# DerEchteKarsten/RayTracer3

Hardware: AMD Instinct MI355X
Metric: Mrays/s (higher is better)
Workload: dtype f32

## Files before the change

### raytracer3_amd/csrc/rt3_device.hpp

```cpp
#pragma once
#include <hip/hip_fp16.h>
#include <hip/hip_runtime.h>
#include <stdint.h>

#define RT3_DEV __device__ __forceinline__

namespace rt3 {

constexpr float kPi = 3.14159265358979323846f;
constexpr float kTau = 6.28318530717958647692f;
constexpr float kInvPi = 0.318309886183790671538f;
constexpr float kHalfPi = 1.57079632679489661923f;
constexpr float kBackgroundDepth = 100000.0f;
constexpr uint32_t kMiss = 0xFFFFFFFFu;
constexpr float kRayTMin = 0.001f;

struct V3 {
    float x, y, z;
};
RT3_DEV V3 v3(float x, float y, float z) { return V3{x, y, z}; }
RT3_DEV V3 operator+(V3 a, V3 b) { return V3{a.x + b.x, a.y + b.y, a.z + b.z}; }
RT3_DEV V3 operator-(V3 a, V3 b) { return V3{a.x - b.x, a.y - b.y, a.z - b.z}; }
RT3_DEV V3 operator*(V3 a, V3 b) { return V3{a.x * b.x, a.y * b.y, a.z * b.z}; }
RT3_DEV V3 operator*(V3 a, float s) { return V3{a.x * s, a.y * s, a.z * s}; }
// ... 511 lines not shown
    const float a[3] = {p00.x, p00.y, p00.z}, bq[3] = {p10.x, p10.y, p10.z}, c[3] = {p01.x, p01.y, p01.z}, dq[3] = {p11.x, p11.y, p11.z};
    float o[3];
#pragma unroll
    for (int k = 0; k < 3; k++) {
        float top = a[k] * (1.0f - fx) + bq[k] * fx, bot = c[k] * (1.0f - fx) + dq[k] * fx;
        o[k] = top * (1.0f - fy) + bot * fy;
    }
    return v3(o[0], o[1], o[2]);
}
RT3_DEV V3 sky_eval(const SceneDev& sc, float u, float v) {
    if (!sc.sky) return v3(0.0f, 0.0f, 0.0f);
    float unused;
    return sky_eval_pdf(sc, u, v, -1, -1, unused);
}
RT3_DEV V3 sky_eval_and_pdf(const SceneDev& sc, float u, float v, float& pdf) {
    int W = (int)sc.sky_w, H = (int)sc.sky_h;
    int ix = (int)(u * (float)W), iy = (int)(v * (float)H);
    ix = ix < 0 ? 0 : (ix > W - 1 ? W - 1 : ix);
    iy = iy < 0 ? 0 : (iy > H - 1 ? H - 1 : iy);
    float pt;
    V3 rad = sky_eval_pdf(sc, u, v, ix, iy, pt);
    float st, ct;
    sincos_2pi(v * 0.5f, st, ct);
    pdf = st > 0.0f ? pt / (2.0f * kPi * kPi * st) : 0.0f;
    return rad;
}
typedef float f32x4_u __attribute__((ext_vector_type(4), aligned(4)));
RT3_DEV uint32_t cdf_find_guided(const float* cdfp, const uint32_t* guide, uint32_t n, float u, float& lo_v, float& hi_v) {
    uint32_t k = (uint32_t)(u * (float)n);
    k = k > n - 1 ? n - 1 : k;
    const uint32_t g = guide[k];
    uint32_t lo = g & 0xFFFFu, hi = g >> 16;
    if (hi - lo <= 2u) {
        const f32x4_u c = *reinterpret_cast<const f32x4_u*>(cdfp + lo);
        const bool s1 = lo < hi && !(c.y > u);
        const bool s2 = s1 && lo + 1u < hi && !(c.z > u);
        lo_v = s2 ? c.z : (s1 ? c.y : c.x);
        hi_v = s2 ? c.w : (s1 ? c.z : c.y);
        return lo + (s1 ? 1u : 0u) + (s2 ? 1u : 0u);
    }
    while (lo < hi) {
        uint32_t mid = (lo + hi) >> 1;
        if (cdfp[mid + 1] > u) hi = mid;
        else lo = mid + 1;
    }
    lo_v = cdfp[lo];
    hi_v = cdfp[lo + 1];
    return lo;
}
struct SkyPick {
    float u, v, sin_theta;
    int x, y;
};
RT3_DEV SkyPick sky_sample_direction(const SceneDev& sc, const float* cdf_marg, const uint32_t* guide_marg, float u0, float u1, V3& dir) {
    uint32_t W = sc.sky_w, H = sc.sky_h;
    float lo, hi;
    uint32_t y = cdf_find_guided(cdf_marg, guide_marg, H, u0, lo, hi);
    float dv = hi > lo ? (u0 - lo) / (hi - lo) : 0.5f;
    const float sx = u1 * (float)W;
    uint32_t k = (uint32_t)sx;
    k = k > W - 1 ? W - 1 : k;
    float xi = sx - (float)k;
    xi = xi < 0.99999994f ? xi : 0.99999994f;
    const uint32_t e = sc.sky_alias[(size_t)y * W + k];
    const float Q = (float)((e & 0xFFFFu) + 1u) * (1.0f / 65536.0f);
    const bool keep = xi < Q;
    const uint32_t x = keep ? k : (e >> 16);
    float du = keep ? xi / Q : (xi - Q) / (1.0f - Q);
    du = du < 0.99999994f ? du : 0.99999994f;
    SkyPick p;
    p.u = ((float)x + du) / (float)W;
    p.v = ((float)y + dv) / (float)H;
    p.x = (int)x;
    p.y = (int)y;
    float st, ct, s2, c2;
    sincos_2pi(p.v * 0.5f, st, ct);
    sincos_2pi(p.u, s2, c2);
    p.sin_theta = st;
    dir = v3((-c2) * st, ct, (-s2) * st);
    return p;
}
RT3_DEV void sky_sample_radiance(const SceneDev& sc, const SkyPick& p, V3& rad, float& pdf) {
    float pt;
    rad = sky_eval_pdf(sc, p.u, p.v, p.x, p.y, pt);
    pdf = p.sin_theta > 0.0f ? pt / (2.0f * kPi * kPi * p.sin_theta) : 0.0f;
}
RT3_DEV void sky_sample(const SceneDev& sc, float u0, float u1, V3& dir, V3& rad, float& pdf) {
    const SkyPick p = sky_sample_direction(sc, sc.cdf_marg, sc.guide_marg, u0, u1, dir);
    sky_sample_radiance(sc, p, rad, pdf);
}

struct LightsDev {
    const float4* rec;
    const uint32_t* cdf;
    const uint32_t* guide;
    const uint32_t* geom_base;
    uint32_t n, guide_shift;
};
RT3_DEV uint32_t light_find(const LightsDev& lt, uint32_t k) {
    const uint32_t c = k >> lt.guide_shift;
    uint32_t lo = lt.guide[c], hi = lt.guide[c + 1];
    while (lo < hi) {
        const uint32_t mid = (lo + hi) >> 1;
        if (lt.cdf[mid] > k) hi = mid;
        else lo = mid + 1;
    }
    return lo;
}

struct Hit {
    float t, u, v;
    uint32_t prim;
};
RT3_DEV float dot_fma(V3 a, V3 b) { return __builtin_fmaf(a.x, b.x, __builtin_fmaf(a.y, b.y, a.z * b.z)); }
RT3_DEV V3 cross_fma(V3 a, V3 b) {
    return V3{__builtin_fmaf(a.y, b.z, -(a.z * b.y)), __builtin_fmaf(a.z, b.x, -(a.x * b.z)), __builtin_fmaf(a.x, b.y, -(a.y * b.x))};
}
RT3_DEV float guarded_inverse(float d) {
    float a = d < 0.0f ? -d : d;
    float g = a < 1e-20f ? (d < 0.0f ? -1e-20f : 1e-20f) : d;
    return 1.0f / g;
}
RT3_DEV bool slab_test(V3 bmin, V3 bmax, V3 o, V3 inv, float tmin, float tbest, float& tn_out) {
    float t0 = (bmin.x - o.x) * inv.x, t1 = (bmax.x - o.x) * inv.x;
    float tn = tmin, tf = tbest;
    float lo = t0 < t1 ? t0 : t1, hi = t0 < t1 ? t1 : t0;
    tn = lo > tn ? lo : tn;
    tf = hi < tf ? hi : tf;
    t0 = (bmin.y - o.y) * inv.y;
    t1 = (bmax.y - o.y) * inv.y;
    lo = t0 < t1 ? t0 : t1;
    hi = t0 < t1 ? t1 : t0;
    tn = lo > tn ? lo : tn;
    tf = hi < tf ? hi : tf;
// ... 29 lines not shown
```

### raytracer3_amd/csrc/rt3_kernels.hip

```cpp
#include <hip/hip_fp16.h>
#include <hip/hip_runtime.h>

#include <type_traits>

#include "rt3_device.hpp"
#include "rt3_internal.hpp"

namespace rt3 {

constexpr int kLdsStack = 12;
constexpr uint32_t kTopFlag = 0x40000000u;
constexpr int kSpill = 64 - kLdsStack;
constexpr uint32_t kMaxSteps = 1u << 20;

constexpr uint32_t kEmptySlot = 0xFFFFFFFFu;
constexpr float kTopPadRel = 2.44140625e-4f;

struct Cand {
    float tn;
    uint32_t ref;
};
__device__ __forceinline__ void cswap(Cand& a, Cand& b) {
    bool sw = b.tn < a.tn;
    float ta = a.tn;
    uint32_t ra = a.ref;
    a.tn = sw ? b.tn : a.tn;
    a.ref = sw ? b.ref : a.ref;
    b.tn = sw ? ta : b.tn;
    b.ref = sw ? ra : b.ref;
}
__device__ __forceinline__ void pin(float4& q) { asm volatile("" : "+v"(q.x), "+v"(q.y), "+v"(q.z), "+v"(q.w)); }
__device__ __forceinline__ V3 cross_exact(V3 a, V3 b) { return V3{(a.y * b.z) - (a.z * b.y), (a.z * b.x) - (a.x * b.z), (a.x * b.y) - (a.y * b.x)}; }
template <bool MASK = false>
__device__ __forceinline__ void tri_test_nb(float4 q0, float4 q1, float4 q2, V3 o, V3 d, float inv_dd, float tmin, Hit& best, const AlphaDev& alpha = AlphaDev{}) {
    const V3 A = v3(q0.x, q0.y, q0.z) - o, B = v3(q0.w, q1.x, q1.y) - o, C = v3(q1.z, q1.w, q2.x) - o;
    const float U = dot_fma(d, cross_exact(B, C)), V = dot_fma(d, cross_exact(C, A)), W = dot_fma(d, cross_exact(A, B));
    const float det = U + (V + W);
    const float inv = 1.0f / det;
    const float w = U * inv, u = V * inv, v = W * inv;
    const float T = __builtin_fmaf(U, dot_fma(A, d), __builtin_fmaf(V, dot_fma(B, d), W * dot_fma(C, d)));
    const float t = (T * inv) * inv_dd;
    const uint32_t prim = __float_as_uint(q2.y);
    constexpr float kEdgeEps = 9.5367431640625e-07f;
    const bool inside = (w >= -kEdgeEps) & (u >= -kEdgeEps) & (v >= -kEdgeEps);
    bool ok = (det != 0.0f) & inside & (t > tmin) & ((t < best.t) | ((t == best.t) & (prim < best.prim)));
    if (MASK && ok && q2.z != 0.0f) ok = alpha_counts(alpha, __float_as_uint(q2.w), q2.z, prim, u, v);
    best.t = ok ? t : best.t;
    best.u = ok ? u : best.u;
    best.v = ok ? v : best.v;
    best.prim = ok ? prim : best.prim;
}

__constant__ uint32_t g_pool_chunk = 256;
__constant__ uint32_t g_refill_lanes = 12;
void set_refill_lanes(uint32_t v) { (void)hipMemcpyToSymbol(HIP_SYMBOL(g_refill_lanes), &v, 4); }
void set_pool_chunk(uint32_t v) { (void)hipMemcpyToSymbol(HIP_SYMBOL(g_pool_chunk), &v, 4); }
static unsigned g_trace_max_blocks = kExtendMaxBlocks;
void set_trace_blocks(uint32_t v) { g_trace_max_blocks = v; }

constexpr uint32_t kTopNodes = kTopCacheNodes;
__device__ __forceinline__ bool load_top(float4* s_top, const float4* __restrict__ top, uint32_t n_top) {
    if (top == nullptr || n_top == 0u) return false;
    n_top = n_top < kTopNodes ? n_top : kTopNodes;
    for (uint32_t i = threadIdx.x; i < 4u * n_top; i += kExtendBlock) s_top[i] = top[i];
    __syncthreads();
    return true;
}

__device__ __forceinline__ bool slab_test_sorted(uint32_t p, uint32_t q, V3 A, V3 B, float tmin, float tbest, float& tn_out) {
    const float nx = __builtin_fmaf((float)(p & 0xFFu), A.x, B.x), ny = __builtin_fmaf((float)((p >> 8) & 0xFFu), A.y, B.y),
                nz = __builtin_fmaf((float)((p >> 16) & 0xFFu), A.z, B.z), fx = __builtin_fmaf((float)(p >> 24), A.x, B.x),
                fy = __builtin_fmaf((float)(q & 0xFFu), A.y, B.y), fz = __builtin_fmaf((float)((q >> 8) & 0xFFu), A.z, B.z);
    const float tn = __builtin_fmaxf(__builtin_fmaxf(nx, ny), __builtin_fmaxf(nz, tmin));
    const float tf = __builtin_fminf(__builtin_fminf(fx, fy), __builtin_fminf(fz, tbest));
    tn_out = tn;
    return tn <= tf;
}

__device__ __forceinline__ bool slab_test_sorted_pad(uint32_t p, uint32_t q, V3 A, V3 B, V3 pad, float tmin, float tbest, float& tn_out) {
    const float nx = __builtin_fmaf((float)(p & 0xFFu), A.x, B.x) - pad.x, ny = __builtin_fmaf((float)((p >> 8) & 0xFFu), A.y, B.y) - pad.y,
                nz = __builtin_fmaf((float)((p >> 16) & 0xFFu), A.z, B.z) - pad.z, fx = __builtin_fmaf((float)(p >> 24), A.x, B.x) + pad.x,
                fy = __builtin_fmaf((float)(q & 0xFFu), A.y, B.y) + pad.y, fz = __builtin_fmaf((float)((q >> 8) & 0xFFu), A.z, B.z) + pad.z;
    const float tn = __builtin_fmaxf(__builtin_fmaxf(nx, ny), __builtin_fmaxf(nz, tmin));
    const float tf = __builtin_fminf(__builtin_fminf(fx, fy), __builtin_fminf(fz, tbest));
    tn_out = tn;
    return tn <= tf;
}

struct LaneRay {
    V3 o, d, inv;
    float tmin, inv_dd;
    Hit best;
    uint32_t cur, leaf_k, index, steps, cn, ct, cl;
    int sp;
    float pay0, pay1;
    float pay2, pay3;
    uint32_t sel_p0, sel_q0, sel_p1, sel_q1;
};

template <int MODE, bool COUNT, int LAYOUT, bool TWO = false, bool RANGE = false, bool MASK = false, typename Finish>
__device__ __forceinline__ void trace_stream(const float4* __restrict__ nodes, const float4* __restrict__ tris,
                                             const float* __restrict__ rays, size_t stride, uint32_t n, uint32_t* __restrict__ work_counter,
                                             uint32_t* __restrict__ lds, Finish finish, bool any_payload = false, bool ext_payload = false, const float4* top_lds = nullptr, bool use_top = false,
                                             const float2* __restrict__ any_contrib = nullptr, const float* __restrict__ any_tmax = nullptr,
                                             const AlphaDev& alpha = AlphaDev{}) {
    constexpr bool ANY = MODE == 1;
    constexpr bool WIDE = LAYOUT == kLayoutWide128;
    constexpr bool WIDEQ = LAYOUT == kLayoutWide64Q || LAYOUT == kLayoutWide48Q;
    constexpr bool C48 = LAYOUT == kLayoutWide48Q;
    uint32_t pool_next = 0, pool_end = 0;
    bool queue_empty = false;
    const uint32_t lane = __lane_id();
    const unsigned long long lanes_below = (1ull << lane) - 1ull;
    const uint32_t n_waves = gridDim.x * (blockDim.x >> 6);
    const uint32_t kRefillLanes = g_refill_lanes,
                   kPoolChunk = (n < 2u * n_waves * g_pool_chunk && g_pool_chunk >= 128u) ? ((g_pool_chunk >> 1) & ~63u) : g_pool_chunk;
    const uint32_t wave_id = blockIdx.x * (blockDim.x >> 6) + (uint32_t)__builtin_amdgcn_readfirstlane((int)(threadIdx.x >> 6));
    bool first_chunk = true;
    uint32_t spill[kSpill];
    LaneRay r;
    r.o = r.d = r.inv = v3(0.0f, 0.0f, 0.0f);
    r.tmin = 0.0f;
    r.inv_dd = 1.0f;
    r.best = Hit{0.0f, 0.0f, 0.0f, kMiss};
    r.cur = r.leaf_k = r.index = r.steps = r.cn = r.ct = r.cl = 0u;
    r.sp = 0;
    r.pay0 = r.pay1 = r.pay2 = r.pay3 = 0.0f;
    r.sel_p0 = r.sel_q0 = r.sel_p1 = r.sel_q1 = 0u;
    bool busy = false;
    V3 tl_o = v3(0.0f, 0.0f, 0.0f), tl_pad = v3(0.0f, 0.0f, 0.0f);
    uint32_t tl_mark = 0u, tl_rec = 0u, tl_base = 0u;
    bool tl_bottom = false;
    auto tl_world = [&]() {
        r.inv = v3(guarded_inverse(r.d.x), guarded_inverse(r.d.y), guarded_inverse(r.d.z));
        tl_o = r.o;
        const float pw = kTopPadRel * __builtin_fmaxf(__builtin_fmaxf(fabsf(r.o.x), fabsf(r.o.y)), fabsf(r.o.z));
        tl_pad = v3(pw * fabsf(r.inv.x), pw * fabsf(r.inv.y), pw * fabsf(r.inv.z));
        tl_bottom = false;
    };
    auto tl_sels = [&]() {
        const uint32_t sx = r.inv.x < 0.0f ? 1u : 0u, sy = r.inv.y < 0.0f ? 1u : 0u, sz = r.inv.z < 0.0f ? 1u : 0u;
        const uint32_t nx = 3u * sx, ny = 1u + 3u * sy, nz = 2u + 3u * sz, fx = 3u - 3u * sx, fy = 4u - 3u * sy, fz = 5u - 3u * sz;
        r.sel_p0 = nx | (ny << 8) | (nz << 16) | (fx << 24);
        r.sel_q0 = fy | (fz << 8);
        r.sel_p1 = r.sel_p0 + 0x02020202u;
        r.sel_q1 = r.sel_q0 + 0x00000202u;
    };
    for (;;) {
        const unsigned long long m_idle = __ballot(!busy);
        if (pool_next >= pool_end && !queue_empty && m_idle != 0ull) {
            uint32_t base = 0;
            if (first_chunk) {
                base = wave_id * kPoolChunk;
                first_chunk = false;
            } else {
                if (lane == 0) base = atomicAdd(work_counter, kPoolChunk);
                base = __builtin_amdgcn_readfirstlane(base);
                const unsigned long long b64 = (unsigned long long)n_waves * kPoolChunk + base;
                base = b64 > 0xFFFFFFFFull ? 0xFFFFFFFFu : (uint32_t)b64;
            }
            queue_empty = base >= n;
            pool_next = base < n ? base : n;
            pool_end = (n - pool_next) > kPoolChunk ? pool_next + kPoolChunk : n;
        }
        if (m_idle != 0ull && pool_next < pool_end && ((uint32_t)__popcll(m_idle) >= kRefillLanes || m_idle == ~0ull)) {
            const uint32_t idx = pool_next + (uint32_t)__popcll(m_idle & lanes_below);
            if (!busy && idx < pool_end) {
                const float4 ro = reinterpret_cast<const float4*>(rays)[idx], rd = reinterpret_cast<const float4*>(rays)[stride + idx];
                r.o = v3(ro.x, ro.y, ro.z);
                r.d = v3(rd.x, rd.y, rd.z);
                const bool payload = ANY ? any_payload : ext_payload;
                r.tmin = payload ? kRayTMin : ro.w;
                r.best = Hit{payload ? kBackgroundDepth : rd.w, 0.0f, 0.0f, kMiss};
                if (RANGE) r.best.t = any_tmax[idx];
                r.pay0 = ro.w;
                r.pay1 = rd.w;
                if (ANY && any_contrib != nullptr) {
                    const float2 c2 = any_contrib[idx];
                    r.pay2 = c2.x;
                    r.pay3 = c2.y;
                }
                r.inv = v3(guarded_inverse(r.d.x), guarded_inverse(r.d.y), guarded_inverse(r.d.z));
                r.inv_dd = 1.0f / dot_fma(r.d, r.d);
                if (LAYOUT == kLayoutWide64Q) {
                    const uint32_t sx = r.inv.x < 0.0f ? 1u : 0u, sy = r.inv.y < 0.0f ? 1u : 0u, sz = r.inv.z < 0.0f ? 1u : 0u;
                    const uint32_t nx = 3u * sx, ny = 1u + 3u * sy, nz = 2u + 3u * sz, fx = 3u - 3u * sx, fy = 4u - 3u * sy, fz = 5u - 3u * sz;
                    r.sel_p0 = nx | (ny << 8) | (nz << 16) | (fx << 24);
                    r.sel_q0 = fy | (fz << 8);
                    r.sel_p1 = r.sel_p0 + 0x02020202u;
                    r.sel_q1 = r.sel_q0 + 0x00000202u;
                }
                r.cur = (LAYOUT == kLayoutWide64Q && use_top) ? kTopFlag : 0u;
                if (TWO) tl_world();
                r.leaf_k = 0u;
                r.sp = 0;
                r.index = idx;
                r.steps = 0u;
                r.cn = r.ct = r.cl = 0u;
                busy = true;
                const float kMaxF = 3.4028234663852886e38f;
                const bool finite_ray = fabsf(r.o.x) <= kMaxF && fabsf(r.o.y) <= kMaxF && fabsf(r.o.z) <= kMaxF && fabsf(r.d.x) <= kMaxF &&
                                        fabsf(r.d.y) <= kMaxF && fabsf(r.d.z) <= kMaxF;
                if (nodes == nullptr || !finite_ray) {
                    finish(r.index, r.best, 0u, 0u, 0u, r.pay0, r.pay1, r.pay2, r.pay3);
                    busy = false;
                }
            }
            const uint32_t taken = (uint32_t)__popcll(m_idle);
            pool_next = pool_next + taken < pool_end ? pool_next + taken : pool_end;
        }
        if (__ballot(busy) == 0ull && pool_next >= pool_end && queue_empty) break;
        if (busy) {
        const bool is_leaf = (r.cur & 0x80000000u) != 0u;
        const uint32_t first = r.cur & 0x0FFFFFFFu, cnt = ((r.cur >> 28) & 7u) + 1u;
        const bool cached = LAYOUT == kLayoutWide64Q && !is_leaf && (r.cur & kTopFlag) != 0u;
        const bool is_inst = TWO && is_leaf && !tl_bottom;
        const bool is_tri = is_leaf && !is_inst;
        const float4* p = is_tri ? tris + 3 * (size_t)(first + r.leaf_k)
                                 : nodes + (WIDE ? 8 : (C48 ? kC48Stride : 4)) * (size_t)(cached ? 0u : (is_inst ? first : r.cur));
        float4 q0, q1, q2, q3, q4, q5, q6, q7;
        if (LAYOUT == kLayoutWide64Q && cached) {
            const float4* t = top_lds + 4 * (r.cur & 0xFFFFu);
            q0 = t[0];
            q1 = t[1];
            q2 = t[2];
            q3 = t[3];
        } else {
            q0 = p[0];
            q1 = p[1];
            q2 = p[2];
            q3 = C48 ? make_float4(0.0f, 0.0f, 0.0f, 0.0f) : p[3];
        }
        if (WIDE) {
            q4 = p[4];
            q5 = p[5];
            q6 = p[6];
            q7 = p[7];
        }
        if (TWO && is_tri) {
            const float4* pm = nodes + 4 * (size_t)(tl_rec + 1u);
            q4 = pm[0];
            q5 = pm[1];
            q6 = pm[2];
            pin(q4); pin(q5); pin(q6);
        }
        pin(q0); pin(q1); pin(q2);
        if (!C48) pin(q3);
        if (WIDE) { pin(q4); pin(q5); pin(q6); pin(q7); }
        bool pop = false, done = false;
        const V3 o = r.o, d = r.d, inv = r.inv;
        const float tmin = r.tmin;
        if (TWO && is_inst) {
            if (COUNT) r.cn++;
            const float mi[12] = {q0.x, q0.y, q0.z, q0.w, q1.x, q1.y, q1.z, q1.w, q2.x, q2.y, q2.z, q2.w};
            const V3 oo = transform_point(mi, o), dd = transform_vector(mi, d);
            r.inv = v3(guarded_inverse(dd.x), guarded_inverse(dd.y), guarded_inverse(dd.z));
            tl_sels();
            const float om = __builtin_fmaxf(__builtin_fmaxf(__builtin_fmaxf(fabsf(o.x), fabsf(o.y)), __builtin_fmaxf(fabsf(o.z), fabsf(oo.x))),
                                             __builtin_fmaxf(fabsf(oo.y), fabsf(oo.z)));
            const float pb = __builtin_fmaf(q3.w, om, q3.z);
            tl_pad = v3(pb * fabsf(r.inv.x), pb * fabsf(r.inv.y), pb * fabsf(r.inv.z));
            tl_o = oo;
            tl_mark = (uint32_t)r.sp;
            tl_rec = first;
            tl_base = __float_as_uint(q3.y);
            tl_bottom = true;
            r.cur = __float_as_uint(q3.x);
        } else if (is_leaf) {
            if (COUNT) r.ct++;
            if (TWO) {
                const float fm[12] = {q4.x, q4.y, q4.z, q4.w, q5.x, q5.y, q5.z, q5.w, q6.x, q6.y, q6.z, q6.w};
                V3 a = v3(q0.x, q0.y, q0.z), b = v3(q0.w, q1.x, q1.y), c = v3(q1.z, q1.w, q2.x);
// ... 150 lines not shown
                    __builtin_amdgcn_sched_barrier(0);
                }
            }
        }
        if (++r.steps >= kMaxSteps) done = true;
        if (done) {
            finish(r.index, r.best, r.cn, r.ct, r.cl, r.pay0, r.pay1, r.pay2, r.pay3);
            busy = false;
        }
        }
    }
}

template <bool COUNT>
struct TraceCounts {
    uint32_t *cnt_nodes, *cnt_tris;
    unsigned long long nodes = 0, tris = 0, lds = 0;
    __device__ __forceinline__ void ray(uint32_t i, uint32_t cn, uint32_t ct, uint32_t cl) {
        if (!COUNT) return;
        if (cnt_nodes) cnt_nodes[i] = cn;
        if (cnt_tris) cnt_tris[i] = ct;
        nodes += cn;
        tris += ct;
        lds += cl;
    }
    __device__ __forceinline__ void add_totals(unsigned long long* totals, unsigned long long* lds_total) {
        if (!COUNT || !totals) return;
        atomicAdd(&totals[0], nodes);
        atomicAdd(&totals[1], tris);
        if (lds_total) atomicAdd(lds_total, lds);
    }
};

template <bool MASK>
struct AlphaArg {
    AlphaDev a;
    __device__ __forceinline__ AlphaDev get() const { return a; }
};
template <>
struct AlphaArg<false> {
    __device__ __forceinline__ AlphaDev get() const { return AlphaDev{}; }
};

template <bool COUNT, int LAYOUT, bool MASK = false>
__global__ __launch_bounds__(kExtendBlock) void k_extend(const float4* __restrict__ nodes, const float4* __restrict__ tris, const float4* __restrict__ top, uint32_t n_top,
                                                         const float* __restrict__ rays, size_t stride,
                                                         const uint32_t* __restrict__ count_ptr, uint32_t count_imm,
                                                         float* __restrict__ hits, uint32_t* __restrict__ cnt_nodes,
                                                         uint32_t* __restrict__ cnt_tris, unsigned long long* __restrict__ totals,
                                                         uint32_t* __restrict__ work_counter, int payload, AlphaArg<MASK> alpha,
                                                         unsigned long long* __restrict__ lds_total) {
    __shared__ uint32_t stack[kLdsStack * kExtendBlock];
    __shared__ float4 s_top[4 * kTopNodes];
    const bool use_top = load_top(s_top, top, n_top);
    const uint32_t n = count_ptr ? *count_ptr : count_imm;
    TraceCounts<COUNT> counts{cnt_nodes, cnt_tris};
    auto finish = [&](uint32_t i, const Hit& h, uint32_t cn, uint32_t ct, uint32_t cl, float, float, float, float) {
        reinterpret_cast<float4*>(hits)[i] = make_float4(h.t, h.u, h.v, __uint_as_float(h.prim));
        counts.ray(i, cn, ct, cl);
    };
    trace_stream<0, COUNT, LAYOUT == kLayoutTwoLevel ? kLayoutWide64Q : LAYOUT, LAYOUT == kLayoutTwoLevel, false, MASK>(
        nodes, tris, rays, stride, n, work_counter, stack + threadIdx.x, finish, false, payload != 0, s_top, use_top, nullptr, nullptr, alpha.get());
    counts.add_totals(totals, lds_total);
}

template <bool COUNT, int LAYOUT, bool RANGE = false, bool MASK = false>
__global__ __launch_bounds__(kExtendBlock) void k_shadow(const float4* __restrict__ nodes, const float4* __restrict__ tris, const float4* __restrict__ top, uint32_t n_top,
                                                         const float* __restrict__ rays, size_t stride,
                                                         const uint32_t* __restrict__ count_ptr, uint32_t count_imm, AlphaArg<MASK> alpha,
                                                         const float* __restrict__ contrib, float* __restrict__ lacc,
                                                         uint32_t* __restrict__ occluded_out, uint32_t* __restrict__ cnt_nodes,
                                                         uint32_t* __restrict__ cnt_tris, unsigned long long* __restrict__ totals,
                                                         uint32_t* __restrict__ work_counter, unsigned long long* __restrict__ lds_total,
                                                         const float* __restrict__ tmax) {
    __shared__ uint32_t stack[kLdsStack * kExtendBlock];
    __shared__ float4 s_top[4 * kTopNodes];
    const bool use_top = load_top(s_top, top, n_top);
    const uint32_t n = count_ptr ? *count_ptr : count_imm;
    TraceCounts<COUNT> counts{cnt_nodes, cnt_tris};
    trace_stream<1, COUNT, LAYOUT == kLayoutTwoLevel ? kLayoutWide64Q : LAYOUT, LAYOUT == kLayoutTwoLevel, RANGE, MASK>(
        nodes, tris, rays, stride, n, work_counter, stack + threadIdx.x,
        [&](uint32_t i, const Hit& h, uint32_t cn, uint32_t ct, uint32_t cl, float c_r, float c_g, float c_b, float c_pid) {
            if (occluded_out) {
                occluded_out[i] = h.prim != kMiss ? 1u : 0u;
            } else if (h.prim == kMiss) {
                float4* L = reinterpret_cast<float4*>(lacc) + __float_as_uint(c_pid);
                float4 v = *L;
                *L = make_float4(v.x + c_r, v.y + c_g, v.z + c_b, 0.0f);
            }
            counts.ray(i, cn, ct, cl);
        },
        occluded_out == nullptr, false, s_top, use_top, occluded_out == nullptr ? reinterpret_cast<const float2*>(contrib) : nullptr, tmax,
        alpha.get());
    counts.add_totals(totals, lds_total);
}

__global__ void k_raygen(GConstDev g, const uint32_t* __restrict__ pixels, uint32_t npix, float* __restrict__ rays, size_t stride) {
    for (uint32_t i = blockIdx.x * blockDim.x + threadIdx.x; i < npix; i += gridDim.x * blockDim.x) {
        uint32_t xy = pixels[i];
        V3 o, d;
        primary_ray(g, xy & 0xFFFFu, xy >> 16, o, d);
        reinterpret_cast<float4*>(rays)[i] = make_float4(o.x, o.y, o.z, 0.0f);
        reinterpret_cast<float4*>(rays)[stride + i] = make_float4(d.x, d.y, d.z, kBackgroundDepth);
    }
}
__global__ void k_gbuffer(SceneDev sc, const uint32_t* __restrict__ pixels, uint32_t npix, uint32_t width,
                          const float* __restrict__ hits, size_t stride, uint4* __restrict__ gbuffer, float* __restrict__ depth) {
    for (uint32_t i = blockIdx.x * blockDim.x + threadIdx.x; i < npix; i += gridDim.x * blockDim.x) {
        uint32_t xy = pixels[i];
        size_t pi = (size_t)(xy >> 16) * width + (xy & 0xFFFFu);
        const float4 hrec = reinterpret_cast<const float4*>(hits)[i];
        uint32_t prim = __float_as_uint(hrec.w);
        if (prim == kMiss) {
            depth[pi] = kBackgroundDepth;
        } else {
            Surface s = hit_info(sc, prim, hrec.y, hrec.z);
            gbuffer[pi] = gbuffer_pack(s);
            depth[pi] = hrec.x;
        }
    }
}

constexpr int kShadeBlock = 512;
struct BlockAppend {
    uint32_t ext, sh;
};
__device__ __forceinline__ BlockAppend block_append2(bool want_ext, bool want_sh, unsigned long long* pair ,
                                                     uint32_t* lds ) {
    constexpr int kWaves = kShadeBlock / 64;
    const uint32_t lane = __lane_id(), wave = threadIdx.x >> 6;
    const unsigned long long m_ext = __ballot(want_ext), m_sh = __ballot(want_sh);
    if (lane == 0) {
        lds[wave] = (uint32_t)__popcll(m_ext);
        lds[kWaves + 1 + wave] = (uint32_t)__popcll(m_sh);
    }
    __syncthreads();
    if (threadIdx.x == 0) {
        uint32_t te = 0, ts = 0;
#pragma unroll
        for (int w = 0; w < kWaves; w++) {
            uint32_t ce = lds[w], cs = lds[kWaves + 1 + w];
            lds[w] = te;
            lds[kWaves + 1 + w] = ts;
            te += ce;
            ts += cs;
// ... 52 lines not shown
}
constexpr float kEmitShadowEnd = 0.9990234375f;

struct ShadeArgs {
    GConstDev g;
    SceneDev sc;
    const uint32_t* pixels;
    const uint2* pixbn;
    uint32_t npix, width;
    FastDiv npix_div;
    uint32_t s0;
    uint32_t bounce;
    const uint4* gbuffer;
    const float* depth;
    const float* in_rays;
    const float* in_hits;
    const float* in_T;
    const uint32_t* in_count;
    uint32_t n_first;
    float* out_rays;
    float* out_T;
    uint32_t* out_count;
    float* sh_rays;
    float* sh_contrib;
    uint32_t* sh_count;
    float* lacc;
    size_t stride;
    LightsDev lights;
    float* sh2_rays;
    float* sh2_contrib;
    float* sh2_tmax;
    uint32_t* sh2_count;
};

template <bool FIRST, bool GLDS, bool EMIT = false>
__global__ __launch_bounds__(kShadeBlock) __attribute__((amdgpu_waves_per_eu(6, 6))) void k_shade(ShadeArgs a) {
    __shared__ uint32_t append_lds[2][(EMIT ? 3 : 2) * (kShadeBlock / 64 + 1)];
    __shared__ ShadeGeomDev s_geoms[GLDS ? kShadeGeomsLds : 1];
    if (GLDS) {
        const uint32_t words = (a.sc.n_geoms < kShadeGeomsLds ? a.sc.n_geoms : kShadeGeomsLds) * (uint32_t)(sizeof(ShadeGeomDev) / 4);
        for (uint32_t k = threadIdx.x; k < words; k += kShadeBlock) reinterpret_cast<uint32_t*>(s_geoms)[k] = reinterpret_cast<const uint32_t*>(a.sc.shade_geoms)[k];
        __syncthreads();
    }
    uint32_t parity = 0;
    constexpr uint32_t kMargRows = 2048;
    __shared__ uint32_t s_guide_marg[kMargRows];
    __shared__ float s_cdf_marg[kMargRows + 4];
    const bool marg_in_lds = (a.g.pad[0] & RT3_FLAG_NEE_SKY) && a.sc.sky != nullptr && a.sc.sky_h <= kMargRows;
    if (marg_in_lds) {
        for (uint32_t k = threadIdx.x; k < a.sc.sky_h; k += kShadeBlock) s_guide_marg[k] = a.sc.guide_marg[k];
        for (uint32_t k = threadIdx.x; k < a.sc.sky_h + 4u; k += kShadeBlock) s_cdf_marg[k] = a.sc.cdf_marg[k];
        __syncthreads();
    }
    const float* cdf_marg = marg_in_lds ? s_cdf_marg : a.sc.cdf_marg;
    const uint32_t* guide_marg = marg_in_lds ? s_guide_marg : a.sc.guide_marg;
    const GConstDev& g = a.g;
    const uint32_t flags = g.pad[0], B = g.bounces, b = a.bounce;
    const uint32_t dims = flags ? 8u : 2u;
    const bool nee = (flags & RT3_FLAG_NEE_SKY) && a.sc.sky != nullptr;
    const bool bnz = (flags & RT3_FLAG_BLUENOISE) && a.sc.bluenoise != nullptr;
    const bool spec = (flags & RT3_FLAG_SPECULAR) != 0u;
    const size_t S = a.stride;
    const uint32_t n = FIRST ? a.n_first : *a.in_count;
    const uint32_t n_round = (n + (kShadeBlock - 1)) & ~(uint32_t)(kShadeBlock - 1);
    for (uint32_t i = blockIdx.x * blockDim.x + threadIdx.x; i < n_round; i += gridDim.x * blockDim.x) {
        bool active = i < n;
        uint32_t pid = 0;
        V3 o = v3(0, 0, 0), d = v3(0, 0, 1), T = v3(1, 1, 1);
        float t = 0.0f, pdf_b = 0.0f;
        Surface surf;
        surf.albedo = surf.emissive = v3(0, 0, 0);
        surf.normal = v3(0, 0, 1);
        surf.roughness = 1.0f;
        surf.metalness = 0.0f;
        uint32_t px = 0, py = 0, sample_in_batch = 0, bn = 0;
        HitRecord hrecord;
        hrecord.rec = make_uint4(0u, 0u, 0u, 0u);
        hrecord.prim = 0u;
        float hbu = 0.0f, hbv = 0.0f;
        float4 ro = make_float4(0.0f, 0.0f, 0.0f, 0.0f), rd = make_float4(0.0f, 0.0f, 1.0f, 0.0f);
        if (!FIRST && active) {
            ro = reinterpret_cast<const float4*>(a.in_rays)[i];
            rd = reinterpret_cast<const float4*>(a.in_rays)[S + i];
        }
        if (active) {
            pid = FIRST ? i : __float_as_uint(rd.w);
            sample_in_batch = fast_div(a.npix_div, pid);
            const uint2 pb = a.pixbn[pid - sample_in_batch * a.npix];
            px = pb.x & 0xFFFFu;
            py = pb.x >> 16;
            bn = pb.y;
        }
        if (FIRST) {
            if (active) {
                size_t pi = (size_t)py * a.width + px;
                float d0 = a.depth[pi];
                if (d0 == kBackgroundDepth) {
                    reinterpret_cast<float4*>(a.lacc)[pid] = make_float4(0.0f, 0.0f, 0.0f, 0.0f);
                    active = false;
                } else {
                    surf = gbuffer_unpack(a.gbuffer[pi]);
                    primary_ray(g, px, py, o, d);
                    t = d0;
                }
            }
        } else if (active) {
            o = v3(ro.x, ro.y, ro.z);
            d = v3(rd.x, rd.y, rd.z);
            T = v3(a.in_T[i], a.in_T[S + i], a.in_T[2 * S + i]);
            pdf_b = ro.w;
            const float4 hrec = reinterpret_cast<const float4*>(a.in_hits)[i];
            uint32_t prim = __float_as_uint(hrec.w);
            if (prim == kMiss) {
                if (nee && pdf_b > 0.0f) {
                    float su, sv;
                    direction_to_equirect_uv(d, su, sv);
                    float pl;
                    V3 rad = sky_eval_and_pdf(a.sc, su, sv, pl);
                    float w = pdf_b / (pdf_b + pl);
                    float4* Lp = reinterpret_cast<float4*>(a.lacc) + pid;
                    float4 lv = *Lp;
                    *Lp = make_float4(lv.x + T.x * (rad.x * w), lv.y + T.y * (rad.y * w), lv.z + T.z * (rad.z * w), 0.0f);
                }
                active = false;
            } else {
                t = hrec.x;
                hbu = hrec.y;
                hbv = hrec.z;
                hrecord = hit_fetch(a.sc, prim);
            }
        }
        bool emit_shadow = false, emit_ext = false;
        V3 wl = v3(0, 1, 0), contrib = v3(0, 0, 0), nd = v3(0, 0, 1), Tn = T;
        float pdf_n = 0.0f;
        bool emit_shadow_e = false;
        V3 wle = v3(0, 1, 0), contrib_e = v3(0, 0, 0);
        float tmax_e = 0.0f;
        if (active) {
            uint32_t seed = rng_seed(px, py, g.frame);
            uint32_t sm = a.s0 + sample_in_batch;
            uint32_t base = (sm * B + b) * dims;
            float u0 = uniform_float(seed, base), u1 = uniform_float(seed, base + 1);
            if (bnz) {
                u0 = bluenoise_shift(u0, bn & 0xFFu);
                u1 = bluenoise_shift(u1, (bn >> 8) & 0xFFu);
            }
            V3 rad = v3(0.0f, 0.0f, 0.0f);
            float pl = 0.0f, cosl = 0.0f;
            SkyPick pick;
            pick.u = pick.v = pick.sin_theta = 0.0f;
            pick.x = pick.y = 0;
            if (nee) {
                float ul0 = uniform_float(seed, base + 3), ul1 = uniform_float(seed, base + 4);
                if (bnz) {
                    ul0 = bluenoise_shift(ul0, (bn >> 16) & 0xFFu);
                    ul1 = bluenoise_shift(ul1, (bn >> 24) & 0xFFu);
                }
                pick = sky_sample_direction(a.sc, cdf_marg, guide_marg, ul0, ul1, wl);
            }
            const bool nee_e = EMIT && b + 1u < B;
            float4 er0 = make_float4(0.0f, 0.0f, 0.0f, 0.0f), er1 = er0, er2 = er0, er3 = er0;
            float eu6 = 0.0f, eu7 = 0.0f;
            if (nee_e) {
                const uint32_t ke = (uint32_t)(uniform_float(seed, base + 5) * 8388608.0f);
                eu6 = uniform_float(seed, base + 6);
                eu7 = uniform_float(seed, base + 7);
                const float4* R = a.lights.rec + 4 * (size_t)light_find(a.lights, ke);
                er0 = R[0];
                er1 = R[1];
                er2 = R[2];
                er3 = R[3];
            }
            if (!FIRST) {
                if (GLDS) surf = hit_finish(a.sc, s_geoms, hrecord, hbu, hbv);
                else surf = hit_finish(a.sc, a.sc.shade_geoms, hrecord, hbu, hbv);
            }
            V3 N = surf.normal;
            if ((flags & RT3_FLAG_FACEFORWARD) && dot(N, d) > 0.0f) N = neg(N);
            if (nee) {
                cosl = dot(N, wl);
                if (cosl > 0.0f) sky_sample_radiance(a.sc, pick, rad, pl);
            }
            V3 b1, b2;
            build_orthonormal_basis(N, b1, b2);
            V3 wi = v3(0.0f, 0.0f, 1.0f), vop = surf.albedo, wo = v3(0.0f, 0.0f, 1.0f);
            float pdf_s = 0.0f;
            bool valid = true;
            Bsdf bs;
            const bool last = b == B - 1;
            if (spec) {
                bs = bsdf_setup(surf.albedo, surf.roughness, surf.metalness);
                wo = v3(-(d.x * b1.x + d.y * b1.y + d.z * b1.z), -(d.x * b2.x + d.y * b2.y + d.z * b2.z), -(d.x * N.x + d.y * N.y + d.z * N.z));
                if (!last) {
                    float u2 = uniform_float(seed, base + 2);
                    valid = bsdf_sample(bs, wo, u0, u1, u2, wi, vop, pdf_s);
                }
            } else if (!last) {
                wi = diffuse_sample(u0, u1);
                pdf_s = wi.z * kInvPi;
            }
            o = v3(o.x + t * d.x, o.y + t * d.y, o.z + t * d.z);
            if (FIRST) {
                reinterpret_cast<float4*>(a.lacc)[pid] = make_float4(T.x * surf.emissive.x, T.y * surf.emissive.y, T.z * surf.emissive.z, 0.0f);
            } else if (surf.emissive.x != 0.0f || surf.emissive.y != 0.0f || surf.emissive.z != 0.0f) {
                V3 le = surf.emissive;
                if (EMIT) {
                    const uint32_t eb = a.lights.geom_base[hrecord.rec.w];
                    if (eb != kMiss) {
                        const float4* R = a.lights.rec + 4 * (size_t)(eb + (hrecord.prim - a.sc.first_prim[hrecord.rec.w]));
                        const float pa = R[0].w;
                        const float4 rn = R[3];
// ... 454 lines not shown
```

Before: 7577.

## Hoist shade-kernel input loads unconditionally and split sky sampling by LDS path

```diff
diff --git a/raytracer3_amd/csrc/rt3_device.hpp b/raytracer3_amd/csrc/rt3_device.hpp
--- a/raytracer3_amd/csrc/rt3_device.hpp
+++ b/raytracer3_amd/csrc/rt3_device.hpp
@@ -587,11 +587,21 @@
     float u, v, sin_theta;
     int x, y;
 };
-RT3_DEV SkyPick sky_sample_direction(const SceneDev& sc, const float* cdf_marg, const uint32_t* guide_marg, float u0, float u1, V3& dir) {
+struct SkyRow {
+    uint32_t y;
+    float dv;
+};
+RT3_DEV SkyRow sky_sample_row(const float* cdf_marg, const uint32_t* guide_marg, uint32_t H, float u0) {
+    float lo, hi;
+    SkyRow r;
+    r.y = cdf_find_guided(cdf_marg, guide_marg, H, u0, lo, hi);
+    r.dv = hi > lo ? (u0 - lo) / (hi - lo) : 0.5f;
+    return r;
+}
+RT3_DEV SkyPick sky_sample_column(const SceneDev& sc, const SkyRow& row, float u1, V3& dir) {
     uint32_t W = sc.sky_w, H = sc.sky_h;
-    float lo, hi;
-    uint32_t y = cdf_find_guided(cdf_marg, guide_marg, H, u0, lo, hi);
-    float dv = hi > lo ? (u0 - lo) / (hi - lo) : 0.5f;
+    const uint32_t y = row.y;
+    const float dv = row.dv;
     const float sx = u1 * (float)W;
     uint32_t k = (uint32_t)sx;
     k = k > W - 1 ? W - 1 : k;
@@ -615,6 +625,9 @@
     dir = v3((-c2) * st, ct, (-s2) * st);
     return p;
 }
+RT3_DEV SkyPick sky_sample_direction(const SceneDev& sc, const float* cdf_marg, const uint32_t* guide_marg, float u0, float u1, V3& dir) {
+    return sky_sample_column(sc, sky_sample_row(cdf_marg, guide_marg, sc.sky_h, u0), u1, dir);
+}
 RT3_DEV void sky_sample_radiance(const SceneDev& sc, const SkyPick& p, V3& rad, float& pdf) {
     float pt;
     rad = sky_eval_pdf(sc, p.u, p.v, p.x, p.y, pt);
diff --git a/raytracer3_amd/csrc/rt3_kernels.hip b/raytracer3_amd/csrc/rt3_kernels.hip
--- a/raytracer3_amd/csrc/rt3_kernels.hip
+++ b/raytracer3_amd/csrc/rt3_kernels.hip
@@ -30,6 +30,7 @@
     b.ref = sw ? ra : b.ref;
 }
 __device__ __forceinline__ void pin(float4& q) { asm volatile("" : "+v"(q.x), "+v"(q.y), "+v"(q.z), "+v"(q.w)); }
+__device__ __forceinline__ void loads_stay_above() { asm volatile("" ::: "memory"); }
 __device__ __forceinline__ V3 cross_exact(V3 a, V3 b) { return V3{(a.y * b.z) - (a.z * b.y), (a.z * b.x) - (a.x * b.z), (a.x * b.y) - (a.y * b.x)}; }
 template <bool MASK = false>
 __device__ __forceinline__ void tri_test_nb(float4 q0, float4 q1, float4 q2, V3 o, V3 d, float inv_dd, float tmin, Hit& best, const AlphaDev& alpha = AlphaDev{}) {
@@ -671,8 +672,6 @@
         for (uint32_t k = threadIdx.x; k < a.sc.sky_h + 4u; k += kShadeBlock) s_cdf_marg[k] = a.sc.cdf_marg[k];
         __syncthreads();
     }
-    const float* cdf_marg = marg_in_lds ? s_cdf_marg : a.sc.cdf_marg;
-    const uint32_t* guide_marg = marg_in_lds ? s_guide_marg : a.sc.guide_marg;
     const GConstDev& g = a.g;
     const uint32_t flags = g.pad[0], B = g.bounces, b = a.bounce;
     const uint32_t dims = flags ? 8u : 2u;
@@ -697,28 +696,38 @@
         hrecord.rec = make_uint4(0u, 0u, 0u, 0u);
         hrecord.prim = 0u;
         float hbu = 0.0f, hbv = 0.0f;
-        float4 ro = make_float4(0.0f, 0.0f, 0.0f, 0.0f), rd = make_float4(0.0f, 0.0f, 1.0f, 0.0f);
-        if (!FIRST && active) {
-            ro = reinterpret_cast<const float4*>(a.in_rays)[i];
-            rd = reinterpret_cast<const float4*>(a.in_rays)[S + i];
-        }
-        if (active) {
-            pid = FIRST ? i : __float_as_uint(rd.w);
-            sample_in_batch = fast_div(a.npix_div, pid);
-            const uint2 pb = a.pixbn[pid - sample_in_batch * a.npix];
-            px = pb.x & 0xFFFFu;
-            py = pb.x >> 16;
-            bn = pb.y;
-        }
+        const uint32_t ic = active ? i : n - 1u;
+        float4 ro = make_float4(0.0f, 0.0f, 0.0f, 0.0f), rd = make_float4(0.0f, 0.0f, 1.0f, 0.0f), hrec = ro;
+        if (!FIRST) {
+            rd = reinterpret_cast<const float4*>(a.in_rays)[S + ic];
+            hrec = reinterpret_cast<const float4*>(a.in_hits)[ic];
+            ro = reinterpret_cast<const float4*>(a.in_rays)[ic];
+            T = v3(a.in_T[ic], a.in_T[S + ic], a.in_T[2 * S + ic]);
+        }
+        pid = FIRST ? ic : __float_as_uint(rd.w);
+        sample_in_batch = fast_div(a.npix_div, pid);
+        const uint2 pb = a.pixbn[pid - sample_in_batch * a.npix];
+        const uint32_t prim = __float_as_uint(hrec.w);
+        const bool hit = !FIRST && active && prim != kMiss;
+        if (!FIRST) hrecord = HitRecord{*(hit ? a.sc.tri_shade + prim : reinterpret_cast<const uint4*>(a.in_hits) + ic), prim};
+        uint4 gtexel = make_uint4(0u, 0u, 0u, 0u);
+        float d0 = 0.0f;
+        px = pb.x & 0xFFFFu;
+        py = pb.x >> 16;
+        bn = pb.y;
+        if (FIRST) {
+            const size_t pi = (size_t)py * a.width + px;
+            d0 = a.depth[pi];
+            gtexel = a.gbuffer[pi];
+        }
+        loads_stay_above();
         if (FIRST) {
             if (active) {
-                size_t pi = (size_t)py * a.width + px;
-                float d0 = a.depth[pi];
                 if (d0 == kBackgroundDepth) {
                     reinterpret_cast<float4*>(a.lacc)[pid] = make_float4(0.0f, 0.0f, 0.0f, 0.0f);
                     active = false;
                 } else {
-                    surf = gbuffer_unpack(a.gbuffer[pi]);
+                    surf = gbuffer_unpack(gtexel);
                     primary_ray(g, px, py, o, d);
                     t = d0;
                 }
@@ -726,10 +735,7 @@
         } else if (active) {
             o = v3(ro.x, ro.y, ro.z);
             d = v3(rd.x, rd.y, rd.z);
-            T = v3(a.in_T[i], a.in_T[S + i], a.in_T[2 * S + i]);
             pdf_b = ro.w;
-            const float4 hrec = reinterpret_cast<const float4*>(a.in_hits)[i];
-            uint32_t prim = __float_as_uint(hrec.w);
             if (prim == kMiss) {
                 if (nee && pdf_b > 0.0f) {
                     float su, sv;
@@ -746,7 +752,6 @@
                 t = hrec.x;
                 hbu = hrec.y;
                 hbv = hrec.z;
-                hrecord = hit_fetch(a.sc, prim);
             }
         }
         bool emit_shadow = false, emit_ext = false;
@@ -775,7 +780,10 @@
                     ul0 = bluenoise_shift(ul0, (bn >> 16) & 0xFFu);
                     ul1 = bluenoise_shift(ul1, (bn >> 24) & 0xFFu);
                 }
-                pick = sky_sample_direction(a.sc, cdf_marg, guide_marg, ul0, ul1, wl);
+                SkyRow row;
+                if (marg_in_lds) row = sky_sample_row(s_cdf_marg, s_guide_marg, a.sc.sky_h, ul0);
+                else row = sky_sample_row(a.sc.cdf_marg, a.sc.guide_marg, a.sc.sky_h, ul0);
+                pick = sky_sample_column(a.sc, row, ul1, wl);
             }
             const bool nee_e = EMIT && b + 1u < B;
             float4 er0 = make_float4(0.0f, 0.0f, 0.0f, 0.0f), er1 = er0, er2 = er0, er3 = er0;
```

After: 7638 (median of 6 runs). No clear change (+0.8%).

## Stage prefetched rays in per-wave LDS ring and shrink LDS stack and top cache

Applied to the files above, without the earlier changes.

```diff
diff --git a/raytracer3_amd/csrc/rt3_kernels.hip b/raytracer3_amd/csrc/rt3_kernels.hip
--- a/raytracer3_amd/csrc/rt3_kernels.hip
+++ b/raytracer3_amd/csrc/rt3_kernels.hip
@@ -8,7 +8,10 @@
 
 namespace rt3 {
 
-constexpr int kLdsStack = 12;
+constexpr int kLdsStack = 8;
+constexpr uint32_t kStageDepth = 32;
+constexpr uint32_t kStageWords = 4u * kStageDepth;
+static_assert(kStageDepth >= 1u && kStageDepth <= 64u, "one prepare run fills at most one entry per lane");
 constexpr uint32_t kTopFlag = 0x40000000u;
 constexpr int kSpill = 64 - kLdsStack;
 constexpr uint32_t kMaxSteps = 1u << 20;
@@ -58,7 +61,9 @@
 static unsigned g_trace_max_blocks = kExtendMaxBlocks;
 void set_trace_blocks(uint32_t v) { g_trace_max_blocks = v; }
 
-constexpr uint32_t kTopNodes = kTopCacheNodes;
+constexpr uint32_t kTopNodes = 64;
+static_assert(kTopNodes <= kTopCacheNodes, "the LDS copy is a prefix of the builder's array");
+constexpr bool kTopPartial = kTopNodes < kTopCacheNodes;
 __device__ __forceinline__ bool load_top(float4* s_top, const float4* __restrict__ top, uint32_t n_top) {
     if (top == nullptr || n_top == 0u) return false;
     n_top = n_top < kTopNodes ? n_top : kTopNodes;
@@ -101,7 +106,8 @@
 template <int MODE, bool COUNT, int LAYOUT, bool TWO = false, bool RANGE = false, bool MASK = false, typename Finish>
 __device__ __forceinline__ void trace_stream(const float4* __restrict__ nodes, const float4* __restrict__ tris,
                                              const float* __restrict__ rays, size_t stride, uint32_t n, uint32_t* __restrict__ work_counter,
-                                             uint32_t* __restrict__ lds, Finish finish, bool any_payload = false, bool ext_payload = false, const float4* top_lds = nullptr, bool use_top = false,
+                                             uint32_t* __restrict__ lds, float4* stage, Finish finish, bool any_payload = false, bool ext_payload = false,
+                                             const float4* top_lds = nullptr, const float4* __restrict__ top_glob = nullptr, bool use_top = false,
                                              const float2* __restrict__ any_contrib = nullptr, const float* __restrict__ any_tmax = nullptr,
                                              const AlphaDev& alpha = AlphaDev{}) {
     constexpr bool ANY = MODE == 1;
@@ -146,42 +152,85 @@
         r.sel_p1 = r.sel_p0 + 0x02020202u;
         r.sel_q1 = r.sel_q0 + 0x00000202u;
     };
+    uint32_t st_head = 0u, st_avail = 0u;
+    const float kStageNaN = __uint_as_float(0x7FC00000u);
     for (;;) {
         const unsigned long long m_idle = __ballot(!busy);
-        if (pool_next >= pool_end && !queue_empty && m_idle != 0ull) {
-            uint32_t base = 0;
-            if (first_chunk) {
-                base = wave_id * kPoolChunk;
-                first_chunk = false;
-            } else {
-                if (lane == 0) base = atomicAdd(work_counter, kPoolChunk);
-                base = __builtin_amdgcn_readfirstlane(base);
-                const unsigned long long b64 = (unsigned long long)n_waves * kPoolChunk + base;
-                base = b64 > 0xFFFFFFFFull ? 0xFFFFFFFFu : (uint32_t)b64;
-            }
-            queue_empty = base >= n;
-            pool_next = base < n ? base : n;
-            pool_end = (n - pool_next) > kPoolChunk ? pool_next + kPoolChunk : n;
-        }
-        if (m_idle != 0ull && pool_next < pool_end && ((uint32_t)__popcll(m_idle) >= kRefillLanes || m_idle == ~0ull)) {
-            const uint32_t idx = pool_next + (uint32_t)__popcll(m_idle & lanes_below);
-            if (!busy && idx < pool_end) {
-                const float4 ro = reinterpret_cast<const float4*>(rays)[idx], rd = reinterpret_cast<const float4*>(rays)[stride + idx];
+        const uint32_t n_idle = (uint32_t)__popcll(m_idle);
+        if (n_idle >= kRefillLanes || m_idle == ~0ull) {
+            if (st_avail < n_idle) {
+                if (pool_next >= pool_end && !queue_empty) {
+                    uint32_t base = 0;
+                    if (first_chunk) {
+                        base = wave_id * kPoolChunk;
+                        first_chunk = false;
+                    } else {
+                        if (lane == 0) base = atomicAdd(work_counter, kPoolChunk);
+                        base = __builtin_amdgcn_readfirstlane(base);
+                        const unsigned long long b64 = (unsigned long long)n_waves * kPoolChunk + base;
+                        base = b64 > 0xFFFFFFFFull ? 0xFFFFFFFFu : (uint32_t)b64;
+                    }
+                    queue_empty = base >= n;
+                    pool_next = base < n ? base : n;
+                    pool_end = (n - pool_next) > kPoolChunk ? pool_next + kPoolChunk : n;
+                }
+                const uint32_t room = kStageDepth - st_avail, left = pool_end - pool_next, n_fill = room < left ? room : left;
+                if (n_fill != 0u) {
+                if (lane < n_fill) {
+                    const uint32_t idx = pool_next + lane;
+                    const float4 ro = reinterpret_cast<const float4*>(rays)[idx], rd = reinterpret_cast<const float4*>(rays)[stride + idx];
+                    float4 ex = make_float4(0.0f, 0.0f, 0.0f, __uint_as_float(idx));
+                    if (ANY && any_contrib != nullptr) {
+                        const float2 c2 = any_contrib[idx];
+                        ex.x = c2.x;
+                        ex.y = c2.y;
+                    }
+                    if (RANGE) ex.z = any_tmax[idx];
+                    const V3 pd = v3(rd.x, rd.y, rd.z);
+                    const V3 pinv = v3(guarded_inverse(pd.x), guarded_inverse(pd.y), guarded_inverse(pd.z));
+                    float pinv_dd = 1.0f / dot_fma(pd, pd);
+                    const float kMaxF = 3.4028234663852886e38f;
+                    const bool finite_ray = fabsf(ro.x) <= kMaxF && fabsf(ro.y) <= kMaxF && fabsf(ro.z) <= kMaxF && fabsf(rd.x) <= kMaxF &&
+                                            fabsf(rd.y) <= kMaxF && fabsf(rd.z) <= kMaxF;
+                    pinv_dd = finite_ray ? pinv_dd : kStageNaN;
+                    uint32_t e = st_head + st_avail + lane;
+                    e = e >= kStageDepth ? e - kStageDepth : e;
+                    stage[e] = ro;
+                    stage[kStageDepth + e] = rd;
+                    stage[2u * kStageDepth + e] = make_float4(pinv.x, pinv.y, pinv.z, pinv_dd);
+                    stage[3u * kStageDepth + e] = ex;
+                }
+                st_avail += n_fill;
+                pool_next += n_fill;
+                __builtin_amdgcn_fence(__ATOMIC_RELEASE, "wavefront");
+                __builtin_amdgcn_wave_barrier();
+                __builtin_amdgcn_fence(__ATOMIC_ACQUIRE, "wavefront");
+                }
+            }
+            const uint32_t give = st_avail < n_idle ? st_avail : n_idle;
+            const uint32_t rank = (uint32_t)__popcll(m_idle & lanes_below);
+            if (!busy && rank < give) {
+                uint32_t e = st_head + rank;
+                e = e >= kStageDepth ? e - kStageDepth : e;
+                const float4 ro = stage[e], rd = stage[kStageDepth + e], ri = stage[2u * kStageDepth + e];
                 r.o = v3(ro.x, ro.y, ro.z);
                 r.d = v3(rd.x, rd.y, rd.z);
                 const bool payload = ANY ? any_payload : ext_payload;
                 r.tmin = payload ? kRayTMin : ro.w;
                 r.best = Hit{payload ? kBackgroundDepth : rd.w, 0.0f, 0.0f, kMiss};
-                if (RANGE) r.best.t = any_tmax[idx];
                 r.pay0 = ro.w;
                 r.pay1 = rd.w;
-                if (ANY && any_contrib != nullptr) {
-                    const float2 c2 = any_contrib[idx];
-                    r.pay2 = c2.x;
-                    r.pay3 = c2.y;
-                }
-                r.inv = v3(guarded_inverse(r.d.x), guarded_inverse(r.d.y), guarded_inverse(r.d.z));
-                r.inv_dd = 1.0f / dot_fma(r.d, r.d);
+                if (ANY) {
+                    const float4 ex = stage[3u * kStageDepth + e];
+                    r.pay2 = ex.x;
+                    r.pay3 = ex.y;
+                    if (RANGE) r.best.t = ex.z;
+                    r.index = __float_as_uint(ex.w);
+                } else {
+                    r.index = __float_as_uint(stage[3u * kStageDepth + e].w);
+                }
+                r.inv = v3(ri.x, ri.y, ri.z);
+                r.inv_dd = ri.w;
                 if (LAYOUT == kLayoutWide64Q) {
                     const uint32_t sx = r.inv.x < 0.0f ? 1u : 0u, sy = r.inv.y < 0.0f ? 1u : 0u, sz = r.inv.z < 0.0f ? 1u : 0u;
                     const uint32_t nx = 3u * sx, ny = 1u + 3u * sy, nz = 2u + 3u * sz, fx = 3u - 3u * sx, fy = 4u - 3u * sy, fz = 5u - 3u * sz;
@@ -194,30 +243,29 @@
                 if (TWO) tl_world();
                 r.leaf_k = 0u;
                 r.sp = 0;
-                r.index = idx;
                 r.steps = 0u;
                 r.cn = r.ct = r.cl = 0u;
                 busy = true;
-                const float kMaxF = 3.4028234663852886e38f;
-                const bool finite_ray = fabsf(r.o.x) <= kMaxF && fabsf(r.o.y) <= kMaxF && fabsf(r.o.z) <= kMaxF && fabsf(r.d.x) <= kMaxF &&
-                                        fabsf(r.d.y) <= kMaxF && fabsf(r.d.z) <= kMaxF;
-                if (nodes == nullptr || !finite_ray) {
+                if (nodes == nullptr || ri.w != ri.w) {
                     finish(r.index, r.best, 0u, 0u, 0u, r.pay0, r.pay1, r.pay2, r.pay3);
                     busy = false;
                 }
             }
-            const uint32_t taken = (uint32_t)__popcll(m_idle);
-            pool_next = pool_next + taken < pool_end ? pool_next + taken : pool_end;
-        }
-        if (__ballot(busy) == 0ull && pool_next >= pool_end && queue_empty) break;
+            st_head += give;
+            st_head = st_head >= kStageDepth ? st_head - kStageDepth : st_head;
+            st_avail -= give;
+        }
+        if (__ballot(busy) == 0ull && st_avail == 0u && pool_next >= pool_end && queue_empty) break;
         if (busy) {
         const bool is_leaf = (r.cur & 0x80000000u) != 0u;
         const uint32_t first = r.cur & 0x0FFFFFFFu, cnt = ((r.cur >> 28) & 7u) + 1u;
-        const bool cached = LAYOUT == kLayoutWide64Q && !is_leaf && (r.cur & kTopFlag) != 0u;
+        const bool in_top = LAYOUT == kLayoutWide64Q && !is_leaf && (r.cur & kTopFlag) != 0u;
+        const bool cached = in_top && (!kTopPartial || (r.cur & 0xFFFFu) < kTopNodes);
         const bool is_inst = TWO && is_leaf && !tl_bottom;
         const bool is_tri = is_leaf && !is_inst;
         const float4* p = is_tri ? tris + 3 * (size_t)(first + r.leaf_k)
                                  : nodes + (WIDE ? 8 : (C48 ? kC48Stride : 4)) * (size_t)(cached ? 0u : (is_inst ? first : r.cur));
+        if (kTopPartial && in_top) p = top_glob + 4 * (size_t)(r.cur & 0xFFFFu);
         float4 q0, q1, q2, q3, q4, q5, q6, q7;
         if (LAYOUT == kLayoutWide64Q && cached) {
             const float4* t = top_lds + 4 * (r.cur & 0xFFFFu);
@@ -474,6 +522,7 @@
                                                          unsigned long long* __restrict__ lds_total) {
     __shared__ uint32_t stack[kLdsStack * kExtendBlock];
     __shared__ float4 s_top[4 * kTopNodes];
+    __shared__ float4 s_stage[(kExtendBlock / 64) * kStageWords];
     const bool use_top = load_top(s_top, top, n_top);
     const uint32_t n = count_ptr ? *count_ptr : count_imm;
     TraceCounts<COUNT> counts{cnt_nodes, cnt_tris};
@@ -482,7 +531,8 @@
         counts.ray(i, cn, ct, cl);
     };
     trace_stream<0, COUNT, LAYOUT == kLayoutTwoLevel ? kLayoutWide64Q : LAYOUT, LAYOUT == kLayoutTwoLevel, false, MASK>(
-        nodes, tris, rays, stride, n, work_counter, stack + threadIdx.x, finish, false, payload != 0, s_top, use_top, nullptr, nullptr, alpha.get());
+        nodes, tris, rays, stride, n, work_counter, stack + threadIdx.x, s_stage + (threadIdx.x >> 6) * kStageWords, finish, false, payload != 0, s_top, top, use_top,
+        nullptr, nullptr, alpha.get());
     counts.add_totals(totals, lds_total);
 }
 
@@ -497,11 +547,12 @@
                                                          const float* __restrict__ tmax) {
     __shared__ uint32_t stack[kLdsStack * kExtendBlock];
     __shared__ float4 s_top[4 * kTopNodes];
+    __shared__ float4 s_stage[(kExtendBlock / 64) * kStageWords];
     const bool use_top = load_top(s_top, top, n_top);
     const uint32_t n = count_ptr ? *count_ptr : count_imm;
     TraceCounts<COUNT> counts{cnt_nodes, cnt_tris};
     trace_stream<1, COUNT, LAYOUT == kLayoutTwoLevel ? kLayoutWide64Q : LAYOUT, LAYOUT == kLayoutTwoLevel, RANGE, MASK>(
-        nodes, tris, rays, stride, n, work_counter, stack + threadIdx.x,
+        nodes, tris, rays, stride, n, work_counter, stack + threadIdx.x, s_stage + (threadIdx.x >> 6) * kStageWords,
         [&](uint32_t i, const Hit& h, uint32_t cn, uint32_t ct, uint32_t cl, float c_r, float c_g, float c_b, float c_pid) {
             if (occluded_out) {
                 occluded_out[i] = h.prim != kMiss ? 1u : 0u;
@@ -512,7 +563,7 @@
             }
             counts.ray(i, cn, ct, cl);
         },
-        occluded_out == nullptr, false, s_top, use_top, occluded_out == nullptr ? reinterpret_cast<const float2*>(contrib) : nullptr, tmax,
+        occluded_out == nullptr, false, s_top, top, use_top, occluded_out == nullptr ? reinterpret_cast<const float2*>(contrib) : nullptr, tmax,
         alpha.get());
     counts.add_totals(totals, lds_total);
 }
```

After: 7554 before, 7530 after. No clear change (-0.3%).
